# rvolden/C3POa

Hardware: AMD Instinct MI355X
Metric: R2C2 reads->consensus/sec (higher is better)
Workload: dtype int32

## Files before the change

c3poa_amd/_lib.py:

```python
import ctypes as C
import os

import numpy as np

_HERE = os.path.dirname(os.path.abspath(__file__))
LIB_PATH = os.environ.get("C3POA_LIB", os.path.join(_HERE, "lib", "libc3poa_hip.so"))
MAX_PEAKS = 256

STAGE_CONK, STAGE_PEAKS, STAGE_POA, STAGE_POLISH, STAGES_ALL = 1, 2, 4, 8, 15
STAGE_QV = 16
QV_GLOBAL, QV_ANCHOR_START, QV_ANCHOR_END = 0, 1, 2
ST_OK, ST_NOT_ASSIGNED, ST_NO_PEAKS, ST_NO_CONSENSUS, ST_TOO_SHORT, ST_LIMIT = range(6)

EXPORTS = ["c3_default_config", "c3_version", "c3_device_count", "c3_warm_device", "c3_create", "c3_destroy", "c3_last_error", "c3_set_splints",
           "c3_batch_upload", "c3_batch_stage", "c3_batch_commit", "c3_batch_assign", "c3_batch_run", "c3_batch_sync", "c3_batch_results", "c3_batch_results_snapshot", "c3_batch_results_fetch", "c3_batch_timing",
           "c3_fetch_track", "c3_fetch_smoothed", "c3_fetch_raw_peaks", "c3_fetch_draft", "c3_fetch_msa2",
           "c3_call_peaks", "c3_poa_msa", "c3_pairwise_consensus", "c3_determine_consensus", "c3_zero_repeats", "c3_scan_splints",
           "c3_reader_open", "c3_reader_open_range", "c3_reader_close", "c3_reader_error", "c3_reader_names_only", "c3_reader_next", "c3_reader_next_set", "c3_reader_noqual", "c3_reader_reserved_bytes", "c3_reader_range_lost", "c3_write_group",
           "c3_scan_adapters", "c3_match_index", "c3_match_index_batch", "c3_demux_indexes", "c3_demux_host",
           "c3_assign_open", "c3_assign_close", "c3_assign_batch", "c3_assign_seen", "c3_write_splint_psl",
           "c3_host_alloc", "c3_host_free", "c3_writer_reset",
           "c3_batch_results_fetch_qv", "c3_batch_results_qv", "c3_batch_qv_timing", "c3_consensus_qv", "c3_consensus_qv_host",
           "c3_write_consensus_fastq",
           "c3_bgzf_create", "c3_bgzf_destroy", "c3_bgzf_bound", "c3_bgzf_compress", "c3_bgzf_compress_host",
# ... 28 lines not shown
                ("sub_beg", C.c_int32 * MAX_PEAKS), ("sub_end", C.c_int32 * MAX_PEAKS)]


RESULT_DTYPE = np.dtype([("status", "<i4"), ("n_peaks", "<i4"), ("n_sub", "<i4"), ("has_front", "<i4"),
                         ("has_tail", "<i4"), ("front_end", "<i4"), ("tail_beg", "<i4"), ("cons_len", "<i4"),
                         ("draft_len", "<i4"), ("n_win", "<i4"), ("peaks", "<i4", (MAX_PEAKS,)),
                         ("sub_beg", "<i4", (MAX_PEAKS,)), ("sub_end", "<i4", (MAX_PEAKS,))])
assert RESULT_DTYPE.itemsize == C.sizeof(ReadResult)


class Timing(C.Structure):
    _fields_ = [(n, C.c_float) for n in ("ms_pack", "ms_conk", "ms_peaks", "ms_poa", "ms_prep", "ms_window",
                                         "ms_stitch", "ms_total")] + \
               [(n, C.c_int64) for n in ("n_reads", "n_bases", "n_windows", "cells_conk", "cells_poa", "cells_polish", "n_poa_redo")] + \
               [(n, C.c_float) for n in ("ms_wall", "ms_host_worklist", "ms_alloc", "ms_host_gap")] + \
               [(n, C.c_int64) for n in ("cells_polish_computed", "n_band_layers", "n_band_fallback", "n_band_mismatch", "n_win_redo", "n_poa_redo16")]


def _fields_dict(t):
    return {f[0]: getattr(t, f[0]) for f in t._fields_}


class _Info(C.Structure):

    def as_dict(self):
        return {k: int(getattr(self, k)) for k, _t in self._fields_}


class QvTiming(C.Structure):
    _fields_ = [("ms_qv", C.c_float)] + [(n, C.c_int64) for n in ("n_reads", "n_pieces", "n_skipped", "band_cells", "edge_hits")]

# ... 1578 lines not shown
```

c3poa_amd/csrc/c3_args.h:

```cpp
#pragma once
#include "c3_dev.h"
#include <cstddef>

struct C3Counters {
  int queue;
  int peaks_queue;
  unsigned long long cells;
  unsigned long long cells_computed;
  unsigned long long zero_cells;
  int poa_ovf;
  int poa_ovf16;
  int n_windows;
  int win_ovf;
  int win_queue2;
  int band_layers, band_fallback;
  int band_mismatch;
  struct { int window, layer, R, q, band_row, full_row, next_row; } verify;
  unsigned long long phases[16];
};
static_assert(offsetof(C3Counters, cells) % 8 == 0 && offsetof(C3Counters, cells_computed) % 8 == 0 &&
              offsetof(C3Counters, zero_cells) % 8 == 0 && offsetof(C3Counters, phases) % 8 == 0, "u64 counters must be 8-byte aligned");

struct ConkArgs {
  C3Batch b; const uint8_t* sp_codes; const int* sp_len; int32_t* track; C3Info* info; C3Counters* cnt;
  int match, mismatch, penalty;
  int n_spl; int32_t* scan;
};
struct PeaksArgs {
  C3Batch b; const int32_t* track; C3Info* info; double* bufA; double* bufB; int32_t* cand; uint8_t* cstate;
  int32_t* raw_peaks; int32_t* n_raw; const int* sp_len; double coef[64]; int64_t maxL; int window, iters, min_dist;
  C3Counters* cnt;
};
struct PoaArgs {
  C3Batch b; C3Info* info; C3Params p; C3Counters* cnt; const int* work; int n_work;
  int* ibase; int* ebase; char* cellsb; uint8_t* bbase; long long* score;
  int Ncap, K, Pcap, cells_cap;
  uint8_t* draft; int32_t* tpos; uint8_t* msa_dbg; const int64_t* msa_off; int* msa_len;
  int rb_span;
  int no2col;
  uint4* desc; int* jump;
  int* pbase;
  int* overflow;
  int* overflow16;
};
#define C3_POA_NI 19
__host__ __device__ inline int c3_poa_far_shift(bool w32) { return w32 ? 0 : 2; }
struct PoaLayout { size_t ints, edges, cells, bases, score, desc, jump, path, total; };
__host__ __device__ inline PoaLayout c3_poa_layout(size_t Ncap, size_t K, int cells_cap, int far_shift, size_t Pcap) {
  PoaLayout l;
  l.ints = sizeof(int) * C3_POA_NI * Ncap; l.edges = sizeof(int) * 3 * Ncap * K;
  l.cells = 2 * (size_t)cells_cap + 16 * (size_t)(cells_cap >> far_shift);
  l.bases = 5 * Ncap; l.score = sizeof(long long) * Ncap; l.desc = sizeof(uint4) * 2 * Ncap;
  l.jump = sizeof(int) * C3_JUMP_LEVELS * Ncap; l.path = sizeof(int) * Pcap;
  l.total = l.ints + l.edges + l.cells + l.bases + l.score + l.desc + l.jump + l.path;
// ... 69 lines not shown
```

c3poa_amd/csrc/c3_stages.hip:

```cpp
#include "c3_host.h"

__global__ void k_summary(const C3Info* info, const int64_t* off, int n, Summary* out) {
  int i = blockIdx.x * blockDim.x + threadIdx.x;
  if (i >= n) return;
  const C3Info* p = &info[i];
  Summary s; s.status = p->status; s.n_sub = p->n_sub; s.max_sub = 0; s.sum_sub = 0; s.max_dang = 0; s.n_peaks = p->n_peaks;
  for (int k = 0; k < p->n_sub; ++k) { int l = p->sub_end[k] - p->sub_beg[k]; s.sum_sub += l; if (l > s.max_sub) s.max_sub = l; }
  int L = (int)(off[i + 1] - off[i]);
  s.front = p->has_front ? p->front_end : 0; s.tail = p->has_tail ? L - p->tail_beg : 0;
  if (p->has_front) s.max_dang = p->front_end;
  if (p->has_tail && L - p->tail_beg > s.max_dang) s.max_dang = L - p->tail_beg;
  out[i] = s;
}

static hipError_t zero_counters(c3_handle* h) { return hipMemsetAsync(h->d_counter.p, 0, sizeof(C3Counters), h->stream); }

static int auto_slots(c3_handle* h, int want, size_t per_slot_bytes, int n_items, int waves_per_cu) {
  int s = want > 0 ? want : h->n_cus * waves_per_cu;
  size_t budget = h->mem_total ? h->mem_total / 3 : ((size_t)64 << 30);
  if (per_slot_bytes > 0) { size_t mx = budget / per_slot_bytes; if ((size_t)s > mx) s = (int)std::max<size_t>(mx, 1); }
  if (s > n_items) s = std::max(n_items, 1);
  return s;
}

// ... 163 lines not shown
  const PoaLayout L = c3_poa_layout(Ncap, K, (int)cells, c3_poa_far_shift(w32), Pcap);
  const int slots = auto_slots(h, h->cfg.slots_poa, L.total, nw, waves_per_cu);
  const size_t S = (size_t)slots;
  HIPCHK(h->s_poa_i.ensure(L.ints * S)); HIPCHK(h->s_poa_nk.ensure(L.edges * S));
  HIPCHK(h->s_poa_cells.ensure(L.cells * S + 256)); HIPCHK(h->s_poa_b.ensure(L.bases * S)); HIPCHK(h->s_poa_sc.ensure(L.score * S));
  HIPCHK(h->s_poa_desc.ensure(L.desc * S)); HIPCHK(h->s_poa_jump.ensure(L.jump * S)); HIPCHK(h->s_poa_path.ensure(L.path * S));
  PoaArgs a; memset(&a, 0, sizeof(a));
  a.b = dev_batch(h); a.info = h->d_info.as<C3Info>(); a.p = dev_params(h->cfg);
  a.cnt = dev_cnt(h); a.work = d_work; a.n_work = nw;
  a.ibase = h->s_poa_i.as<int>(); a.ebase = h->s_poa_nk.as<int>(); a.cellsb = h->s_poa_cells.as<char>();
  a.bbase = h->s_poa_b.as<uint8_t>(); a.score = h->s_poa_sc.as<long long>();
  a.Ncap = Ncap; a.K = K; a.Pcap = Pcap; a.cells_cap = (int)cells; a.desc = h->s_poa_desc.as<uint4>(); a.jump = h->s_poa_jump.as<int>();
  a.pbase = h->s_poa_path.as<int>(); a.overflow = d_overflow; a.overflow16 = d_overflow16;
  if (const char* e = getenv("C3_DEBUG_POA_RBSPAN")) a.rb_span = std::max(3300, atoi(e));
  a.no2col = getenv("C3_DEBUG_POA_NO2COL") != nullptr;
  a.draft = h->d_draft.as<uint8_t>(); a.tpos = h->d_tpos.as<int32_t>();
  a.msa_dbg = nullptr; a.msa_off = nullptr; a.msa_len = nullptr;
  if (h->debug_msa) { a.msa_dbg = h->d_msa.as<uint8_t>(); a.msa_off = h->d_msa_off.as<int64_t>(); a.msa_len = h->d_msa_len.as<int>(); }
  DBG("poa: nw=%d Ncap=%d K=%d cells=%lld slots=%d (%.1f MB per slot)%s\n", nw, Ncap, K, cells, slots, L.total / 1048576.0, d_overflow ? "" : (d_overflow16 ? " [full-size pass]" : " [32-bit pass]"));
  c3k_launch_poa(&a, slots, w32 ? 1 : 0, wide_ring, h->stream);
  HIPCHK(hipGetLastError());
  return 0;
}

static int run_poa(c3_handle* h) {
  const int nw = (int)h->work.size();
  HIPCHK(h->d_draft.ensure((size_t)h->total + 64)); HIPCHK(h->d_tpos.ensure(sizeof(int32_t) * (size_t)h->total + 64));
  HIPCHK(h->d_cons.ensure((size_t)h->total + 64));
  HIPCHK(hipMemsetAsync(h->d_tpos.p, 0xff, sizeof(int32_t) * (size_t)h->total, h->stream));
  if (nw == 0) return 0;
// ... 7 lines not shown
  const double nodes_typ = (double)max_q * (1.0 + 0.15 * std::max(0, max_ns - 1));
  int Ncap = (int)std::min<double>(Ncap_full, 1.3 * nodes_typ + 256);
  long long cells = std::min<long long>(cells_full, (long long)(1.5 * nodes_typ * (2 * w + 12)) + 4096);
  if (const char* e_ = getenv("C3_DEBUG_POA_SMALL")) { Ncap = std::min(Ncap_full, std::max(64, atoi(e_))); cells = std::min<long long>(cells_full, 16LL * Ncap); }
  if (h->debug_msa) {
    std::vector<int64_t> mo(h->n + 1, 0);
    for (int i = 0; i < h->n; ++i) mo[i + 1] = mo[i] + (int64_t)h->sum[i].n_sub * (h->sum[i].sum_sub + 2);
    HIPCHK(h->d_msa.ensure((size_t)mo[h->n] + 64)); HIPCHK(h->d_msa_off.ensure(sizeof(int64_t) * (h->n + 1))); HIPCHK(h->d_msa_len.ensure(sizeof(int) * h->n));
    HIPCHK(hipMemcpyAsync(h->d_msa_off.p, mo.data(), sizeof(int64_t) * (h->n + 1), hipMemcpyHostToDevice, h->stream));
    HIPCHK(hipMemsetAsync(h->d_msa_len.p, 0, sizeof(int) * h->n, h->stream));
    HIPCHK(hipStreamSynchronize(h->stream));
  }
  HIPCHK(h->d_overflow.ensure(sizeof(int) * 2 * (size_t)nw));
  C3Counters* dc = dev_cnt(h);
  HIPCHK(zero_cnt(h, &dc->queue)); HIPCHK(zero_cnt(h, &dc->cells)); HIPCHK(zero_cnt(h, &dc->poa_ovf)); HIPCHK(zero_cnt(h, &dc->poa_ovf16));
  HIPCHK(zero_cnt(h, &dc->phases));
  int wide_ring = (max_q > 1792 || 2 * w + 1 + 24 > 128) ? 1 : 0;
  if (const char* e_ = getenv("C3_DEBUG_POA_WIDE")) wide_ring = atoi(e_) ? 1 : 0;
  int* ovA = h->d_overflow.as<int>(); int* ovB = h->d_overflow.as<int>() + nw;
  int rc = launch_poa(h, h->d_work.as<int>(), nw, Ncap, K, Pcap, cells, ovA, ovB, 24, wide_ring);
  if (rc) return rc;
  h->n_poa_redo = 0; h->n_poa_redo16 = 0;
  C3Counters c;
  HIPCHK(read_counters(h, &c));
  if (c.poa_ovf > 0) {
    h->n_poa_redo = c.poa_ovf;
    HIPCHK(zero_cnt(h, &dc->queue));
    if ((rc = launch_poa(h, ovA, c.poa_ovf, Ncap_full, K, Pcap, cells_full, nullptr, ovB, 24, wide_ring))) return rc;
    HIPCHK(read_counters(h, &c));
  }
// ... 188 lines not shown
  float ms_prep = 0, ms_win = 0, ms_st = 0;
  if (stages & (C3_STAGE_POA | C3_STAGE_POLISH)) {
    DBG("run: conk+peaks launched\n");
    if ((rc = fetch_summary(h))) return rc;
    DBG("run: work list ready (%zu reads)\n", h->work.size());
    HIPCHK(hipEventRecord(t3, h->stream));
    if (stages & C3_STAGE_POA) {
      if ((rc = run_poa(h))) return rc;
    }
    HIPCHK(hipEventRecord(t4, h->stream));
    if (stages & C3_STAGE_POA) {
      C3Counters c;
      HIPCHK(read_counters(h, &c));
      if (!h->work.empty()) h->tm.cells_poa = (int64_t)(c.zero_cells + c.cells);
      h->tm.n_poa_redo = h->n_poa_redo; h->tm.n_poa_redo16 = h->n_poa_redo16;
      DBG("run: poa done\n");
      HIPCHK(hipEventElapsedTime(&ms, t3, t4)); h->tm.ms_poa = ms;
    }
    if (stages & C3_STAGE_POLISH) { if ((rc = run_polish(h, &ms_prep, &ms_win, &ms_st))) return rc; }
  }
  if (stages & C3_STAGE_QV) { if ((rc = run_qv(h))) return rc; }
  HIPCHK(hipStreamSynchronize(h->stream));
  DBG("run: done\n");
  HIPCHK(hipGetLastError());
  if (stages & C3_STAGE_CONK) { HIPCHK(hipEventElapsedTime(&ms, t0, t1)); h->tm.ms_conk = ms; }
  if (stages & C3_STAGE_PEAKS) { HIPCHK(hipEventElapsedTime(&ms, t1, t2)); h->tm.ms_peaks = ms; }
  if (stages & C3_STAGE_POLISH) { h->tm.ms_prep = ms_prep; h->tm.ms_window = ms_win; h->tm.ms_stitch = ms_st; }
  h->tm.ms_total = h->tm.ms_conk + h->tm.ms_peaks + h->tm.ms_poa + h->tm.ms_prep + h->tm.ms_window + h->tm.ms_stitch;
  h->tm.ms_wall = std::chrono::duration<float, std::milli>(std::chrono::steady_clock::now() - wall0).count();
  h->tm.ms_alloc = (float)(c3h::g_alloc_ms - alloc0);
// ... 6 lines not shown
```

c3poa_amd/csrc/k_poa.hip:

```cpp
#include "c3_dev.h"
#include "c3_args.h"
#include "c3_launch.h"
#include <type_traits>

#define WSYNC() __syncthreads()
#define EI(v, k) ((size_t)(k) * (size_t)c.Ncap + (size_t)(v))
#define SRC 0
#define SNK 1


struct Ctx {
  int* I; int* E; char* C; uint8_t* B8; long long* score_; uint4* desc_; int* jump_; int* path_;
  int K, n, Ncap, cells_cap;
  int far_shift;
  int osel;
  int rb_span;
  int two_col;
  const uint32_t* pk;
#ifdef C3_DEBUG_PUNT
  unsigned long long* dbg;
#endif
#define CTX_I(name, k) __device__ __forceinline__ int* name() const { return I + (size_t)(k) * Ncap; }
  CTX_I(n_in, 0) CTX_I(n_out, 1) CTX_I(grp, 2) CTX_I(index, 5) CTX_I(gfirst, 6) CTX_I(glast, 7)
  CTX_I(rem, 8) CTX_I(mpl, 9) CTX_I(mpr, 10) CTX_I(rowm, 11)  CTX_I(anchor, 14) CTX_I(col, 15)
  CTX_I(col2t, 16) CTX_I(nxt, 17) CTX_I(foff, 18)
#undef CTX_I
  __device__ __forceinline__ int* order() const { return I + (size_t)(3 + osel) * Ncap; }
  __device__ __forceinline__ int* order2() const { return I + (size_t)(4 - osel) * Ncap; }
  __device__ __forceinline__ int* in_from() const { return E; }
  __device__ __forceinline__ int* out_to() const { return E + (size_t)Ncap * K; }
  __device__ __forceinline__ int* out_w() const { return E + 2 * (size_t)Ncap * K; }
  __device__ __forceinline__ int far_cap() const { return cells_cap >> far_shift; }
// ... 120 lines not shown
#endif
__device__ __forceinline__ int maxu16(int a, int b) { int d; asm C3_ASMV("v_max_u16 %0, %1, %2" : "=v"(d) : "v"(a), "v"(b)); return d; }
__device__ __forceinline__ int minu16(int a, int b) { int d; asm C3_ASMV("v_min_u16 %0, %1, %2" : "=v"(d) : "v"(a), "v"(b)); return d; }
__device__ __forceinline__ int cv_16to9(int v, int b8) { return v >= ZLO16 ? (int)((unsigned)(v - BIAS16 + b8) << 6) : NEGS; }
__device__ __forceinline__ int cv_9to16(int x9, int b8, int& bad) {
  if (x9 <= NEGS / 2) return NEG16;
  const int r = (x9 >> 6) - b8 + BIAS16;
  if (r < GLO16 || r > 62000) bad = 1;
  return r;
}


__device__ void poa_sweep_desc(Ctx& c, int lane, int Q, bool qlds, const int PR) {
  const int n = c.n;
  int* hops = c.col();
  for (int c0 = ((n - 1) >> 6) << 6; c0 >= 0; c0 -= 64) {
    const int idx = c0 + lane;
    const bool live = idx < n;
    const int v = live ? c.order()[idx] : SNK;
    const int nin = live ? c.n_in()[v] : 0, nout = live ? c.n_out()[v] : 0;
    int bw = INT32_MIN, bt = SNK;
    unsigned far = 0;
    for (int k = 0; __builtin_amdgcn_ballot_w64(k < nout) != 0; ++k) {
      if (k < nout) {
        const int t = c.out_to()[EI(v, k)], ww = c.out_w()[EI(v, k)];
        if (ww > bw) { bw = ww; bt = t; }
        if (t == SNK || c.index()[t] - idx > PR - 1) far = 1;
      }
    }
    unsigned p[4] = {0, 0, 0, 0};
#pragma unroll
    for (int k = 0; k < 4; ++k) if (k < nin) p[k] = (unsigned)c.index()[c.in_from()[EI(v, k)]];
    int d = (v == SNK) ? 0 : 1, ptr = (v == SNK || !live) ? -1 : c.index()[bt];
    if (ptr >= c0 + 64) { d += hops[ptr]; ptr = -1; }
    for (int r = 0; r < 6 && __builtin_amdgcn_ballot_w64(ptr >= 0) != 0; ++r) {
      const int src = (max(ptr, c0) - c0) << 2;
      const int dd = __builtin_amdgcn_ds_bpermute(src, d), pp = __builtin_amdgcn_ds_bpermute(src, ptr);
      if (ptr >= 0) { d += dd; ptr = pp; }
    }
    if (live) {
      hops[idx] = d;
      uint4 A; A.x = (unsigned)v;
      A.y = (p[0] % PR) | ((p[1] % PR) << 4) | ((p[2] % PR) << 8) | ((p[3] % PR) << 12);
      A.z = (unsigned)c.base()[v] | ((unsigned)min(nin, 255) << 8) | (far << 16) | ((unsigned)(nin > 4) << 17);
      A.z |= ((unsigned)(qlds && nin == 1 && (int)p[0] == idx - 1 && v != SRC && v != SNK) << 18) | ((unsigned)(v == SNK) << 19);
      A.w = (unsigned)(Q - (d - 1));
      uint4 B; B.x = p[0]; B.y = p[1]; B.z = p[2]; B.w = p[3];
      c.descA()[idx] = A; c.descB()[idx] = B;
    }
    WSYNC();
  }
}

template <bool W32, bool DEF, bool WIDE>
__device__ int poa_align(Ctx& c, const C3Params& P, int qb, int Q, int lane, long long* cells PHA) {
  constexpr int PR = WIDE ? 3 : C3_NARROW_PR, PW = WIDE ? C3_WIDE_PW : 128, PWT = PADL + PW + PADR, NCHMAX = PW / 64;
  constexpr int RING_CELLS = WIDE ? RING_CELLS_W : RING_CELLS_N, PQW = WIDE ? PQW_W : PQW_N;
  static_assert(PR * PWT == RING_CELLS, "ring geometry");
  unsigned* const Lqpk = WIDE ? &L.qpk[0] : (unsigned*)&L.ring[3 * RING_CELLS_N];
  const int K = c.K, n = c.n;
// ... 20 lines not shown
    for (int i = lane; i < PQW && from + 16 * i < Q; i += 64) {
      const long long b0 = (long long)qb + from + 16 * i;
      const unsigned w0 = c.pk[b0 >> 4], w1 = c.pk[(b0 >> 4) + 1];
      Lqpk[i] = __builtin_amdgcn_alignbit(w1, w0, (unsigned)(b0 & 15) * 2);
    }
  };
  if (qlds) stage_query(0);
  if (!W32) { unsigned* r32 = (unsigned*)&L.ring[0]; for (int i = lane; i < 3 * RING_CELLS / 2; i += 64) r32[i] = NEG16 | (NEG16 << 16); }
  WSYNC();
  PH_MARK(0)
  int u_beg = 0, u_end = -1, u_left = 0, u_right = 0, u_ncell = 0;
  int u_b8 = 0;
  int u_nfar = 0;
  int pH = NEG16, pE1 = NEG16, pE2 = NEG16;
  bool pv_ok = false;
  int gacc = 0xffff;
  int punt = 0;
  const int lane4 = lane * 4;
  unsigned short* const LH = &L.ring[0]; unsigned short* const LE1 = &L.ring[RING_CELLS]; unsigned short* const LE2 = &L.ring[2 * RING_CELLS];
#ifdef C3_EXP_SBAND
#define UNI(x)
#else
#define UNI(x) asm volatile("" : "+v"(x))
#endif
#ifdef C3_PHASE_PROF
  unsigned long long row_t0 = __builtin_readcyclecounter();
#endif
  int slot = PR - 1;
  for (int ib = 0; ib < n; ib += 64) {
  uint4 dA = c.descA()[min(ib + lane, n - 1)], dB = c.descB()[min(ib + lane, n - 1)];
  asm volatile("" : "+v"(dA.x), "+v"(dA.y), "+v"(dA.z), "+v"(dA.w), "+v"(dB.x), "+v"(dB.y), "+v"(dB.z), "+v"(dB.w));
  const int cnt = min(64, n - ib);
  for (int li = 0; li < cnt; ++li) {
    const int idx = ib + li;
    slot = slot == PR - 1 ? 0 : slot + 1;
    const int fl = __builtin_amdgcn_readlane(dA.z, li);
    if ((fl >> 19) & 1) { pv_ok = false; continue; }
    const int qr = __builtin_amdgcn_readlane(dA.w, li);
    const int vb = fl & 0xff;
    const bool far = W32 || ((fl >> 16) & 1);
    if (WIDE && qr + w + 72 > qwb + PQW * 16 && qwb + PQW * 16 < Q) {
      qwb = max(0, qr - w - 320) & ~15;
      WSYNC(); stage_query(qwb); WSYNC();
    }
#define C3_BAND_OF_ROW_ABOVE \
      UNI(u_beg); UNI(u_end); UNI(u_left); UNI(u_right); UNI(u_ncell); \
      const bool nonempty = u_end >= u_beg; \
      const int mplv = nonempty ? u_left + 1 : INT32_MAX / 2, mprv = nonempty ? u_right + 1 : 0; \
      const int beg = max(max(0, min(mplv, qr) - w), u_beg); \
      int end = min(min(Q, max(mprv, qr) + w), u_end + 1); \
      end = max(end, beg - 1); \
      const int wd = end - beg + 1, sh = beg - u_beg;
    if (!W32 && ((fl >> 18) & 1) && pv_ok) {
      C3_BAND_OF_ROW_ABOVE
      if (__builtin_amdgcn_ballot_w64(((int)((unsigned)(wd - 1) < 64u) & (int)(wd + sh <= 64) & ((int)(sh >= 1) | (int)(u_end - u_beg < 63)) & (int)(u_ncell + 64 <= c.cells_cap) & (int)(!far || u_nfar + 64 <= c.far_cap()) & (int)(!WIDE || (max(beg - 1, 0) >= qwb && end <= qwb + PQW * 16))) != 0) != 0) {
        const int ro = u_ncell;
        const int j = beg + lane;
        const bool act = lane < wd;
        const int jq = max(j - 1, 0) - (WIDE ? qwb : 0);
        const unsigned qw_ = Lqpk[min(jq >> 4, PQW - 1)];
        const int a_p = lane4 + sh * 4, a_d = a_p - 4;
        const int hd = __builtin_amdgcn_ds_bpermute(a_d, pH), hp = __builtin_amdgcn_ds_bpermute(a_p, pH);
        const int e1p = __builtin_amdgcn_ds_bpermute(a_p, pE1), e2p = __builtin_amdgcn_ds_bpermute(a_p, pE2);
        const int qc = (int)((qw_ >> ((jq & 15) * 2)) & 3);
        const int M = hd + ((vb == qc) ? mt8 + 2 : mm8 + 2);
        const int E1t = maxu16(hp - (oe1_8 - 1), e1p - e1_8);
        const int E2t = maxu16(hp - (oe2_8 - 2), e2p - e2_8);
        const int E1c = E1t & ~7, E2c = E2t & ~7;
        const int k2 = maxu16(maxu16(M, E1c + 1), E2c);
        const int ht = k2 & ~7;
// ... 11 lines not shown
        const int rb = __builtin_amdgcn_readlane(s3, 63);
        const unsigned long long mxm = __ballot(htm == rb);
        const int left = beg + __builtin_ctzll(mxm), right = beg + (63 - __builtin_clzll(mxm));
        pH = maxu16(act ? h : NEG16, FLOOR16); pE1 = act ? E1c : NEG16; pE2 = act ? E2c : NEG16;
        int nb8 = u_b8;
        if ((unsigned)(rb - RB_LO16) > (unsigned)c.rb_span) {
          const int m1 = rb - BIAS16, fl1 = FLOOR16 + max(m1, 0);
          nb8 += m1; punt |= (int)(rb < GLO16);
          pH = act ? maxu16(h, fl1) - m1 : NEG16; pE1 = act ? maxu16(E1c, fl1) - m1 : NEG16; pE2 = act ? maxu16(E2c, fl1) - m1 : NEG16;
        }
        gacc = minu16(gacc, pH - (ZHI16 + 1));
#ifdef C3_DEBUG_PUNT
        if (pH > ZHI16 && pH < GLO16) { atomicAdd(c.dbg + 8, 1ull); atomicMax(c.dbg + 9, ((unsigned long long)(65535 - pH) << 40) | ((unsigned long long)idx << 16) | ((unsigned long long)lane << 8) | (unsigned long long)(wd & 255)); atomicMax(c.dbg + 10, ((unsigned long long)(65535 - pH) << 40) | ((unsigned long long)(unsigned short)rb << 16) | (unsigned)(sh & 255) << 8 | (unsigned)(u_end - u_beg + 1)); }
#endif
        c.D8()[(unsigned)(ro + lane)] = (uint8_t)d;
        { const int cb = slot * PWT + PADL + lane;
          LH[cb] = (unsigned short)pH; LE1[cb] = (unsigned short)pE1; LE2[cb] = (unsigned short)pE2;
#pragma unroll
          for (int f = 1; f < NCHMAX; ++f) { LH[cb + 64 * f] = NEG16; LE1[cb + 64 * f] = NEG16; LE2[cb + 64 * f] = NEG16; }
        }
        if (lane == 0) {
          L.meta[slot] = make_int4(beg, end, left, right); L.base8[slot] = nb8;
          int off = 3 * idx; UNI(off);
          int* rm = c.rowm() + off; rm[0] = beg; rm[1] = end; rm[2] = ro;
        }
        if (far) {
          const int fo = wave_first(u_nfar);
          if (act) { c.H()[fo + lane] = cv_16to9(pH, nb8); c.E1()[fo + lane] = cv_16to9(pE1, nb8); c.E2()[fo + lane] = cv_16to9(pE2, nb8); }
          if (lane == 0) { c.mpl()[idx] = left; c.mpr()[idx] = right; c.foff()[idx] = fo; }
          u_nfar = fo + wave_first(wd);
        }
        u_beg = beg; u_end = end; u_left = left; u_right = right; u_ncell = ro + wd; u_b8 = nb8;
#ifdef C3_PHASE_PROF
        { unsigned long long t_ = __builtin_readcyclecounter(); ph_acc_[8] += t_ - row_t0; row_t0 = t_; ph_acc_[12] += 1; }
#endif
        continue;
      }
    }
    if (!WIDE && !W32 && ((fl >> 18) & 1) && c.two_col) {
      C3_BAND_OF_ROW_ABOVE
      if (__builtin_amdgcn_ballot_w64(((int)((unsigned)(wd - 65) < 64u) & (int)((unsigned)(u_end - u_beg) < (unsigned)PW) & (int)(u_ncell + 128 <= c.cells_cap) & (int)(!far || u_nfar + 128 <= c.far_cap())) != 0) != 0) {
        const int ro = u_ncell;
        int c0l = 2 * lane; UNI(c0l);
        const bool act0 = c0l < wd, act1 = c0l + 1 < wd;
        const int j0 = beg + c0l;
        const int jq0 = max(j0 - 1, 0), jq1 = j0;
        const unsigned qw0 = Lqpk[min(jq0 >> 4, PQW - 1)], qw1 = Lqpk[min(jq1 >> 4, PQW - 1)];
        const int rx = (slot == 0 ? PR - 1 : slot - 1) * PWT + PADL + sh + c0l;
        const int hd0 = LH[rx - 1], hp0 = LH[rx], hp1 = LH[rx + 1];
        const int e1p0 = LE1[rx], e1p1 = LE1[rx + 1], e2p0 = LE2[rx], e2p1 = LE2[rx + 1];
        const int qc0 = (int)((qw0 >> ((jq0 & 15) * 2)) & 3), qc1 = (int)((qw1 >> ((jq1 & 15) * 2)) & 3);
        const int M0 = hd0 + ((vb == qc0) ? mt8 + 2 : mm8 + 2), M1 = hp0 + ((vb == qc1) ? mt8 + 2 : mm8 + 2);
        const int E1t0 = maxu16(hp0 - (oe1_8 - 1), e1p0 - e1_8), E1t1 = maxu16(hp1 - (oe1_8 - 1), e1p1 - e1_8);
        const int E2t0 = maxu16(hp0 - (oe2_8 - 2), e2p0 - e2_8), E2t1 = maxu16(hp1 - (oe2_8 - 2), e2p1 - e2_8);
        const int E1c0 = E1t0 & ~7, E2c0 = E2t0 & ~7, E1c1 = E1t1 & ~7, E2c1 = E2t1 & ~7;
        const int k20 = maxu16(maxu16(M0, E1c0 + 1), E2c0), k21 = maxu16(maxu16(M1, E1c1 + 1), E2c1);
// ... 75 lines not shown
#pragma unroll
      for (int k = 0; k < NP; ++k) {
        const bool has = k < nin;
        const int b = has ? m_[k].x : BIGB, e = has ? m_[k].y : -BIGB;
        pb_[k] = b;
        dk_[k] = has ? b8_[k] - b8_[0] : 0;
        dabs = max(dabs, max(dk_[k], -dk_[k]));
        minb = min(minb, b); maxe = max(maxe, e + 1); wmax = max(wmax, e - b);
        const bool ne = e >= b;
        mplv = ne ? min(mplv, m_[k].z + 1) : mplv; mprv = ne ? max(mprv, m_[k].w + 1) : mprv;
      }
      const int beg = max(max(0, min(mplv, qr) - w), minb);
      int end = min(min(Q, max(mprv, qr) + w), maxe);
      end = max(end, beg - 1);
      const int wd = end - beg + 1;
      if (__builtin_amdgcn_ballot_w64(((int)((unsigned)(wd - 1) < (unsigned)(64 * NCH)) & (int)(wmax < PW) & (int)(dabs < 2048) & (int)(u_ncell + 64 * NCH <= c.cells_cap) & (int)(!far || u_nfar + 64 * NCH <= c.far_cap()) & (int)(!WIDE || (max(beg - 1, 0) >= qwb && end <= qwb + PQW * 16))) != 0) == 0) return false;
      const int ro = u_ncell;
      const int W8 = wave_first(b8_[0]);
      int cM[NP], c1o[NP], c1x[NP], c2o[NP], c2x[NP], sb_[NP];
#pragma unroll
      for (int k = 0; k < NP; ++k) {
        cM[k] = dk_[k] + (3 - k);
        c1o[k] = dk_[k] - oe1_8 + (7 - 2 * k); c1x[k] = dk_[k] - e1_8 + (6 - 2 * k);
        c2o[k] = dk_[k] - oe2_8 + (7 - 2 * k); c2x[k] = dk_[k] - e2_8 + (6 - 2 * k);
        sb_[k] = sl_[k] * PWT + PADL - pb_[k];
      }
      int carry1 = 0, carry2 = 0, prev_ht = NEG16;
      int best = 0, left = 0, right = 0;
      int cH[NCH], cE1[NCH], cE2[NCH];
#pragma unroll
      for (int ch = 0; ch < NCH; ++ch) {
// ... 254 lines not shown
        if (c0 + 64 >= wd) { for (int f = 64; c0 + f < PW; f += 64) { LH[cb + f] = NEG16; LE1[cb + f] = NEG16; LE2[cb + f] = NEG16; } }
        if (c0 == 0) { gH = vH; gE1 = vE1; gE2 = vE2; }
      }
      if (cmx > best) { best = cmx; const unsigned long long mm = __ballot(htm == cmx); bl = beg + c0 + __builtin_ctzll(mm); br = beg + c0 + 63 - __builtin_clzll(mm); }
      else if (cmx == best) { const unsigned long long mm = __ballot(htm == cmx); if (mm) br = beg + c0 + 63 - __builtin_clzll(mm); }
    }
    if (!W32 && __builtin_amdgcn_ballot_w64(bad != 0) != 0) punt |= 2;
    const int left = wd > 0 ? bl : 0, right = wd > 0 ? br : 0;
    if (lane == 0) {
      L.meta[slot] = make_int4(beg, end, left, right); L.base8[slot] = Wg;
      { int* rm = c.rowm() + 3 * idx; rm[0] = beg; rm[1] = end | (ty << 28); rm[2] = ro; }
      if (far) { c.mpl()[idx] = left; c.mpr()[idx] = right; }
      if (toglobal || ovf) c.foff()[idx] = fo;
    }
    u_beg = beg; u_end = end; u_left = left; u_right = right; u_ncell = ncell; u_b8 = Wg;
#ifdef C3_PHASE_PROF
    { unsigned long long t_ = __builtin_readcyclecounter(); ph_acc_[11] += t_ - row_t0; row_t0 = t_; }
#endif
    pH = gH; pE1 = gE1; pE2 = gE2; pv_ok = inl && wd <= 64;
  }
  }
  WSYNC();
  *cells += wave_first(u_ncell);
  PH_MARK(1)
#ifdef C3_DEBUG_PUNT
  if (!W32 && lane == 0) { if (punt) atomicAdd(c.dbg + 14, 1ull); if (__builtin_amdgcn_ballot_w64((unsigned)(gacc & 0xffff) < (unsigned)(GLO16 - ZHI16 - 1)) != 0) atomicAdd(c.dbg + 15, 1ull); }
#endif
  if (!W32 && (punt != 0 || __builtin_amdgcn_ballot_w64((unsigned)(gacc & 0xffff) < (unsigned)(GLO16 - ZHI16 - 1)) != 0)) return -5;
  int bi = -1, bs = INT32_MIN;
  for (int k = 0; k < c.n_in()[SNK]; ++k) {
// ... 220 lines not shown
}

#ifndef C3_POA_WAVES
#define C3_POA_WAVES 6
#endif
template <bool W32, bool DEF, bool WIDE>
__global__ __launch_bounds__(64, C3_POA_WAVES) void k_poa(PoaArgs a) {
  const int lane = wave_lane();
  const int slot = blockIdx.x;
  Ctx c;
  const size_t N = (size_t)a.Ncap;
  c.I = a.ibase + (size_t)slot * C3_POA_NI * N; c.path_ = a.pbase + (size_t)slot * a.Pcap; c.E = a.ebase + (size_t)slot * 3 * N * a.K;
  c.far_shift = c3_poa_far_shift(W32);
  c.C = a.cellsb + (size_t)slot * c3_poa_layout(N, a.K, a.cells_cap, c.far_shift, a.Pcap).cells; c.B8 = a.bbase + (size_t)slot * 5 * N;
  c.score_ = a.score + (size_t)slot * N; c.desc_ = a.desc + (size_t)slot * 2 * N; c.jump_ = a.jump + (size_t)slot * C3_JUMP_LEVELS * N;
  c.K = a.K; c.Ncap = a.Ncap; c.cells_cap = a.cells_cap; c.osel = 0; c.rb_span = a.rb_span > 0 ? a.rb_span : RB_HI16 - RB_LO16; c.two_col = !a.no2col;
#ifdef C3_DEBUG_PUNT
  c.dbg = a.cnt->phases;
#endif
  PH_DECL

  for (;;) {
    int wi = 0;
    if (lane == 0) wi = atomicAdd(&a.cnt->queue, 1);
    wi = wave_first(wi);
    if (wi >= a.n_work) break;
    const int rid = a.work[wi];
    C3Info* info = &a.info[rid];
    const int ns = info->n_sub;
    const int64_t off = a.b.off[rid];
    c.pk = a.b.pk + a.b.woff[rid];
    uint8_t* draft = a.draft + off;
    int32_t* tpos = a.tpos + off;
    const uint8_t* qual = a.b.qual + off;
    long long cells = 0;
// ... 166 lines not shown
    const bool to16 = punted || a.overflow == nullptr;
    int* const olist = to16 ? a.overflow16 : a.overflow;
    const bool redo = fail == 2 && olist != nullptr;
    if (lane == 0) {
      if (redo) olist[atomicAdd(to16 ? &a.cnt->poa_ovf16 : &a.cnt->poa_ovf, 1)] = rid;
      else {
        info->draft_len = C;
        if (fail) { info->status = C3_ST_LIMIT; info->draft_len = 0; }
        else if (C == 0) info->status = C3_ST_NO_CONSENSUS;
        atomicAdd(&a.cnt->cells, (unsigned long long)cells);
      }
    }
    WSYNC();
  }
  PH_FLUSH(a.cnt->phases)
}

extern "C" void c3k_launch_poa(const PoaArgs* a, int slots, int wide32, int wide_ring, hipStream_t stream) {
  const C3Params& p = a->p;
  const bool def = p.poa_match == 5 && p.poa_mismatch == 4 && p.o1 == 4 && p.e1 == 2 && p.o2 == 24 && p.e2 == 1;
#define C3_POA_LAUNCH(W, D, R) hipLaunchKernelGGL((k_poa<W, D, R>), dim3(slots), dim3(64), 0, stream, *a)
  if (wide32) { if (def) C3_POA_LAUNCH(true, true, false); else C3_POA_LAUNCH(true, false, false); }
  else if (wide_ring) { if (def) C3_POA_LAUNCH(false, true, true); else C3_POA_LAUNCH(false, false, true); }
  else { if (def) C3_POA_LAUNCH(false, true, false); else C3_POA_LAUNCH(false, false, false); }
#undef C3_POA_LAUNCH
}
```

include/c3poa.h:

```cpp
#ifndef C3POA_H
#define C3POA_H
#include <stdint.h>

#ifdef __cplusplus
extern "C" {
#endif

#define C3_MAX_PEAKS 256

typedef enum {
  C3_E_OK = 0,
  C3_E_NO_DEVICE = -1,
  C3_E_HIP = -2,
  C3_E_ARG = -3,
  C3_E_NOMEM = -4,
  C3_E_STATE = -5,
  C3_E_LIMIT = -6,
  C3_E_DATA = -7
} c3_err;

typedef enum {
  C3_ST_OK = 0,
  C3_ST_NOT_ASSIGNED = 1,
  C3_ST_NO_PEAKS = 2,
// ... 32 lines not shown

typedef struct {
  float ms_pack, ms_conk, ms_peaks, ms_poa, ms_prep, ms_window, ms_stitch, ms_total;
  int64_t n_reads, n_bases, n_windows;
  int64_t cells_conk, cells_poa, cells_polish;
  int64_t n_poa_redo;
  float ms_wall;
  float ms_host_worklist;
  float ms_alloc;
  float ms_host_gap;
  int64_t cells_polish_computed;
  int64_t n_band_layers, n_band_fallback;
  int64_t n_band_mismatch;
  int64_t n_win_redo;
  int64_t n_poa_redo16;
} c3_timing;

typedef struct c3_handle c3_handle;

void c3_default_config(c3_config* cfg);
const char* c3_version(void);
int c3_device_count(void);
int c3_warm_device(int device);

int c3_create(const c3_config* cfg, c3_handle** out);
void c3_destroy(c3_handle* h);
const char* c3_last_error(const c3_handle* h);

int c3_set_splints(c3_handle* h, int n, const char* cat, const int64_t* off);

// ... 263 lines not shown
```

Before: 429,800.

## Skip LDS ring writes for chain rows and precompute block capacity checks

```diff
diff --git a/c3poa_amd/_lib.py b/c3poa_amd/_lib.py
--- a/c3poa_amd/_lib.py
+++ b/c3poa_amd/_lib.py
@@ -66,7 +66,8 @@
                                          "ms_stitch", "ms_total")] + \
                [(n, C.c_int64) for n in ("n_reads", "n_bases", "n_windows", "cells_conk", "cells_poa", "cells_polish", "n_poa_redo")] + \
                [(n, C.c_float) for n in ("ms_wall", "ms_host_worklist", "ms_alloc", "ms_host_gap")] + \
-               [(n, C.c_int64) for n in ("cells_polish_computed", "n_band_layers", "n_band_fallback", "n_band_mismatch", "n_win_redo", "n_poa_redo16")]
+               [(n, C.c_int64) for n in ("cells_polish_computed", "n_band_layers", "n_band_fallback", "n_band_mismatch", "n_win_redo", "n_poa_redo16",
+                                         "n_poa_flush", "n_poa_ring_skips")]
 
 
 def _fields_dict(t):
diff --git a/c3poa_amd/csrc/c3_args.h b/c3poa_amd/csrc/c3_args.h
--- a/c3poa_amd/csrc/c3_args.h
+++ b/c3poa_amd/csrc/c3_args.h
@@ -10,6 +10,8 @@
   unsigned long long zero_cells;
   int poa_ovf;
   int poa_ovf16;
+  unsigned long long poa_flush;
+  unsigned long long poa_skip;
   int n_windows;
   int win_ovf;
   int win_queue2;
@@ -19,7 +21,7 @@
   unsigned long long phases[16];
 };
 static_assert(offsetof(C3Counters, cells) % 8 == 0 && offsetof(C3Counters, cells_computed) % 8 == 0 &&
-              offsetof(C3Counters, zero_cells) % 8 == 0 && offsetof(C3Counters, phases) % 8 == 0, "u64 counters must be 8-byte aligned");
+              offsetof(C3Counters, zero_cells) % 8 == 0 && offsetof(C3Counters, poa_flush) % 8 == 0 && offsetof(C3Counters, phases) % 8 == 0, "u64 counters must be 8-byte aligned");
 
 struct ConkArgs {
   C3Batch b; const uint8_t* sp_codes; const int* sp_len; int32_t* track; C3Info* info; C3Counters* cnt;
@@ -38,6 +40,7 @@
   uint8_t* draft; int32_t* tpos; uint8_t* msa_dbg; const int64_t* msa_off; int* msa_len;
   int rb_span;
   int no2col;
+  int ring_all;
   uint4* desc; int* jump;
   int* pbase;
   int* overflow;
diff --git a/c3poa_amd/csrc/c3_stages.hip b/c3poa_amd/csrc/c3_stages.hip
--- a/c3poa_amd/csrc/c3_stages.hip
+++ b/c3poa_amd/csrc/c3_stages.hip
@@ -201,6 +201,7 @@
   a.pbase = h->s_poa_path.as<int>(); a.overflow = d_overflow; a.overflow16 = d_overflow16;
   if (const char* e = getenv("C3_DEBUG_POA_RBSPAN")) a.rb_span = std::max(3300, atoi(e));
   a.no2col = getenv("C3_DEBUG_POA_NO2COL") != nullptr;
+  a.ring_all = getenv("C3_DEBUG_POA_RINGALL") != nullptr;
   a.draft = h->d_draft.as<uint8_t>(); a.tpos = h->d_tpos.as<int32_t>();
   a.msa_dbg = nullptr; a.msa_off = nullptr; a.msa_len = nullptr;
   if (h->debug_msa) { a.msa_dbg = h->d_msa.as<uint8_t>(); a.msa_off = h->d_msa_off.as<int64_t>(); a.msa_len = h->d_msa_len.as<int>(); }
@@ -238,6 +239,7 @@
   HIPCHK(h->d_overflow.ensure(sizeof(int) * 2 * (size_t)nw));
   C3Counters* dc = dev_cnt(h);
   HIPCHK(zero_cnt(h, &dc->queue)); HIPCHK(zero_cnt(h, &dc->cells)); HIPCHK(zero_cnt(h, &dc->poa_ovf)); HIPCHK(zero_cnt(h, &dc->poa_ovf16));
+  HIPCHK(zero_cnt(h, &dc->poa_flush)); HIPCHK(zero_cnt(h, &dc->poa_skip));
   HIPCHK(zero_cnt(h, &dc->phases));
   int wide_ring = (max_q > 1792 || 2 * w + 1 + 24 > 128) ? 1 : 0;
   if (const char* e_ = getenv("C3_DEBUG_POA_WIDE")) wide_ring = atoi(e_) ? 1 : 0;
@@ -456,6 +458,7 @@
       HIPCHK(read_counters(h, &c));
       if (!h->work.empty()) h->tm.cells_poa = (int64_t)(c.zero_cells + c.cells);
       h->tm.n_poa_redo = h->n_poa_redo; h->tm.n_poa_redo16 = h->n_poa_redo16;
+      h->tm.n_poa_flush = (int64_t)c.poa_flush; h->tm.n_poa_ring_skips = (int64_t)c.poa_skip;
       DBG("run: poa done\n");
       HIPCHK(hipEventElapsedTime(&ms, t3, t4)); h->tm.ms_poa = ms;
     }
diff --git a/c3poa_amd/csrc/k_poa.hip b/c3poa_amd/csrc/k_poa.hip
--- a/c3poa_amd/csrc/k_poa.hip
+++ b/c3poa_amd/csrc/k_poa.hip
@@ -16,6 +16,7 @@
   int osel;
   int rb_span;
   int two_col;
+  int ring_all;
   const uint32_t* pk;
 #ifdef C3_DEBUG_PUNT
   unsigned long long* dbg;
@@ -166,6 +167,7 @@
 __device__ void poa_sweep_desc(Ctx& c, int lane, int Q, bool qlds, const int PR) {
   const int n = c.n;
   int* hops = c.col();
+  int cand_hi = 0;
   for (int c0 = ((n - 1) >> 6) << 6; c0 >= 0; c0 -= 64) {
     const int idx = c0 + lane;
     const bool live = idx < n;
@@ -184,6 +186,9 @@
 #pragma unroll
     for (int k = 0; k < 4; ++k) if (k < nin) p[k] = (unsigned)c.index()[c.in_from()[EI(v, k)]];
     int d = (v == SNK) ? 0 : 1, ptr = (v == SNK || !live) ? -1 : c.index()[bt];
+    const int cand = (int)(live && qlds && nin == 1 && (int)p[0] == idx - 1 && v != SRC && v != SNK);
+    const bool regs_only = nout == 1 && ptr == idx + 1 && wave_shl1(cand, cand_hi) != 0 && !c.ring_all;
+    cand_hi = wave_bcast(cand, 0);
     if (ptr >= c0 + 64) { d += hops[ptr]; ptr = -1; }
     for (int r = 0; r < 6 && __builtin_amdgcn_ballot_w64(ptr >= 0) != 0; ++r) {
       const int src = (max(ptr, c0) - c0) << 2;
@@ -195,7 +200,7 @@
       uint4 A; A.x = (unsigned)v;
       A.y = (p[0] % PR) | ((p[1] % PR) << 4) | ((p[2] % PR) << 8) | ((p[3] % PR) << 12);
       A.z = (unsigned)c.base()[v] | ((unsigned)min(nin, 255) << 8) | (far << 16) | ((unsigned)(nin > 4) << 17);
-      A.z |= ((unsigned)(qlds && nin == 1 && (int)p[0] == idx - 1 && v != SRC && v != SNK) << 18) | ((unsigned)(v == SNK) << 19);
+      A.z |= ((unsigned)cand << 18) | ((unsigned)(v == SNK) << 19) | ((unsigned)!regs_only << 20);
       A.w = (unsigned)(Q - (d - 1));
       uint4 B; B.x = p[0]; B.y = p[1]; B.z = p[2]; B.w = p[3];
       c.descA()[idx] = A; c.descB()[idx] = B;
@@ -246,6 +251,7 @@
   int u_nfar = 0;
   int pH = NEG16, pE1 = NEG16, pE2 = NEG16;
   bool pv_ok = false;
+  bool ring_stale = false;
   int gacc = 0xffff;
   int punt = 0;
   const int lane4 = lane * 4;
@@ -263,11 +269,15 @@
   uint4 dA = c.descA()[min(ib + lane, n - 1)], dB = c.descB()[min(ib + lane, n - 1)];
   asm volatile("" : "+v"(dA.x), "+v"(dA.y), "+v"(dA.z), "+v"(dA.w), "+v"(dB.x), "+v"(dB.y), "+v"(dB.z), "+v"(dB.w));
   const int cnt = min(64, n - ib);
+#define C3_BLOCK_ROOM if (!W32 && __builtin_amdgcn_ballot_w64(((c.cells_cap - 64 * PW - u_ncell) | (c.far_cap() - 64 * PW - u_nfar)) < 0) != 0) dA.z |= 1u << 21;
+#define C3_ROW_ROOM(t, cells) { t |= (c.cells_cap - (cells) - u_ncell) | (far ? c.far_cap() - (cells) - u_nfar : 0); asm volatile("" : "+v"(t)); }
+  C3_BLOCK_ROOM
   for (int li = 0; li < cnt; ++li) {
     const int idx = ib + li;
     slot = slot == PR - 1 ? 0 : slot + 1;
     const int fl = __builtin_amdgcn_readlane(dA.z, li);
-    if ((fl >> 19) & 1) { pv_ok = false; continue; }
+    if ((fl >> 19) & 1) { pv_ok = false; ring_stale = false; continue; }
+    const bool tight = (fl >> 21) & 1;
     const int qr = __builtin_amdgcn_readlane(dA.w, li);
     const int vb = fl & 0xff;
     const bool far = W32 || ((fl >> 16) & 1);
@@ -285,7 +295,10 @@
       const int wd = end - beg + 1, sh = beg - u_beg;
     if (!W32 && ((fl >> 18) & 1) && pv_ok) {
       C3_BAND_OF_ROW_ABOVE
-      if (__builtin_amdgcn_ballot_w64(((int)((unsigned)(wd - 1) < 64u) & (int)(wd + sh <= 64) & ((int)(sh >= 1) | (int)(u_end - u_beg < 63)) & (int)(u_ncell + 64 <= c.cells_cap) & (int)(!far || u_nfar + 64 <= c.far_cap()) & (int)(!WIDE || (max(beg - 1, 0) >= qwb && end <= qwb + PQW * 16))) != 0) != 0) {
+      int qt = (wd - 1) | (u_beg + 63 - end) | ((sh - 1) & (u_beg + 62 - u_end));
+      if (WIDE) qt |= (max(beg - 1, 0) - qwb) | (qwb + PQW * 16 - end);
+      if (tight) C3_ROW_ROOM(qt, 64)
+      if (__builtin_amdgcn_ballot_w64(qt >= 0) != 0) {
         const int ro = u_ncell;
         const int j = beg + lane;
         const bool act = lane < wd;
@@ -327,16 +340,21 @@
         if (pH > ZHI16 && pH < GLO16) { atomicAdd(c.dbg + 8, 1ull); atomicMax(c.dbg + 9, ((unsigned long long)(65535 - pH) << 40) | ((unsigned long long)idx << 16) | ((unsigned long long)lane << 8) | (unsigned long long)(wd & 255)); atomicMax(c.dbg + 10, ((unsigned long long)(65535 - pH) << 40) | ((unsigned long long)(unsigned short)rb << 16) | (unsigned)(sh & 255) << 8 | (unsigned)(u_end - u_beg + 1)); }
 #endif
         c.D8()[(unsigned)(ro + lane)] = (uint8_t)d;
-        { const int cb = slot * PWT + PADL + lane;
-          LH[cb] = (unsigned short)pH; LE1[cb] = (unsigned short)pE1; LE2[cb] = (unsigned short)pE2;
-#pragma unroll
-          for (int f = 1; f < NCHMAX; ++f) { LH[cb + 64 * f] = NEG16; LE1[cb + 64 * f] = NEG16; LE2[cb + 64 * f] = NEG16; }
-        }
         if (lane == 0) {
-          L.meta[slot] = make_int4(beg, end, left, right); L.base8[slot] = nb8;
           int off = 3 * idx; UNI(off);
           int* rm = c.rowm() + off; rm[0] = beg; rm[1] = end; rm[2] = ro;
         }
+        ring_stale = !((fl >> 20) & 1);
+        if (!ring_stale) {
+          const int cb = slot * PWT + PADL + lane;
+          LH[cb] = (unsigned short)pH; LE1[cb] = (unsigned short)pE1; LE2[cb] = (unsigned short)pE2;
+#pragma unroll
+          for (int f = 1; f < NCHMAX; ++f) { LH[cb + 64 * f] = NEG16; LE1[cb + 64 * f] = NEG16; LE2[cb + 64 * f] = NEG16; }
+          if (lane == 0) { L.meta[slot] = make_int4(beg, end, left, right); L.base8[slot] = nb8; }
+        }
+#ifdef C3_PHASE_PROF
+        else if (lane == 0) L.base8[6] = L.base8[6] + 1;
+#endif
         if (far) {
           const int fo = wave_first(u_nfar);
           if (act) { c.H()[fo + lane] = cv_16to9(pH, nb8); c.E1()[fo + lane] = cv_16to9(pE1, nb8); c.E2()[fo + lane] = cv_16to9(pE2, nb8); }
@@ -350,9 +368,20 @@
         continue;
       }
     }
+    if (!W32 && ring_stale) {
+      ring_stale = false;
+      const int pslot = slot == 0 ? PR - 1 : slot - 1;
+      const int cb = pslot * PWT + PADL + lane;
+      LH[cb] = (unsigned short)pH; LE1[cb] = (unsigned short)pE1; LE2[cb] = (unsigned short)pE2;
+#pragma unroll
+      for (int f = 1; f < NCHMAX; ++f) { LH[cb + 64 * f] = NEG16; LE1[cb + 64 * f] = NEG16; LE2[cb + 64 * f] = NEG16; }
+      if (lane == 0) { L.meta[pslot] = make_int4(u_beg, u_end, u_left, u_right); L.base8[pslot] = u_b8; L.base8[7] = L.base8[7] + 1; }
+    }
     if (!WIDE && !W32 && ((fl >> 18) & 1) && c.two_col) {
       C3_BAND_OF_ROW_ABOVE
-      if (__builtin_amdgcn_ballot_w64(((int)((unsigned)(wd - 65) < 64u) & (int)((unsigned)(u_end - u_beg) < (unsigned)PW) & (int)(u_ncell + 128 <= c.cells_cap) & (int)(!far || u_nfar + 128 <= c.far_cap())) != 0) != 0) {
+      int qt = (wd - 65) | (128 - wd) | (u_end - u_beg) | (u_beg + (PW - 1) - u_end);
+      if (tight) C3_ROW_ROOM(qt, 128)
+      if (__builtin_amdgcn_ballot_w64(qt >= 0) != 0) {
         const int ro = u_ncell;
         int c0l = 2 * lane; UNI(c0l);
         const bool act0 = c0l < wd, act1 = c0l + 1 < wd;
@@ -458,7 +487,10 @@
       int end = min(min(Q, max(mprv, qr) + w), maxe);
       end = max(end, beg - 1);
       const int wd = end - beg + 1;
-      if (__builtin_amdgcn_ballot_w64(((int)((unsigned)(wd - 1) < (unsigned)(64 * NCH)) & (int)(wmax < PW) & (int)(dabs < 2048) & (int)(u_ncell + 64 * NCH <= c.cells_cap) & (int)(!far || u_nfar + 64 * NCH <= c.far_cap()) & (int)(!WIDE || (max(beg - 1, 0) >= qwb && end <= qwb + PQW * 16))) != 0) == 0) return false;
+      int qt = (wd - 1) | (64 * NCH - wd) | (PW - 1 - wmax) | (2047 - dabs);
+      if (WIDE) qt |= (max(beg - 1, 0) - qwb) | (qwb + PQW * 16 - end);
+      if (tight) C3_ROW_ROOM(qt, 64 * NCH)
+      if (__builtin_amdgcn_ballot_w64(qt >= 0) == 0) return false;
       const int ro = u_ncell;
       const int W8 = wave_first(b8_[0]);
       int cM[NP], c1o[NP], c1x[NP], c2o[NP], c2x[NP], sb_[NP];
@@ -743,6 +775,7 @@
       if (toglobal || ovf) c.foff()[idx] = fo;
     }
     u_beg = beg; u_end = end; u_left = left; u_right = right; u_ncell = ncell; u_b8 = Wg;
+    C3_BLOCK_ROOM
 #ifdef C3_PHASE_PROF
     { unsigned long long t_ = __builtin_readcyclecounter(); ph_acc_[11] += t_ - row_t0; row_t0 = t_; }
 #endif
@@ -993,11 +1026,12 @@
   c.far_shift = c3_poa_far_shift(W32);
   c.C = a.cellsb + (size_t)slot * c3_poa_layout(N, a.K, a.cells_cap, c.far_shift, a.Pcap).cells; c.B8 = a.bbase + (size_t)slot * 5 * N;
   c.score_ = a.score + (size_t)slot * N; c.desc_ = a.desc + (size_t)slot * 2 * N; c.jump_ = a.jump + (size_t)slot * C3_JUMP_LEVELS * N;
-  c.K = a.K; c.Ncap = a.Ncap; c.cells_cap = a.cells_cap; c.osel = 0; c.rb_span = a.rb_span > 0 ? a.rb_span : RB_HI16 - RB_LO16; c.two_col = !a.no2col;
+  c.K = a.K; c.Ncap = a.Ncap; c.cells_cap = a.cells_cap; c.osel = 0; c.rb_span = a.rb_span > 0 ? a.rb_span : RB_HI16 - RB_LO16; c.two_col = !a.no2col; c.ring_all = a.ring_all;
 #ifdef C3_DEBUG_PUNT
   c.dbg = a.cnt->phases;
 #endif
   PH_DECL
+  if (lane == 0) { L.base8[6] = 0; L.base8[7] = 0; }
 
   for (;;) {
     int wi = 0;
@@ -1194,6 +1228,10 @@
     WSYNC();
   }
   PH_FLUSH(a.cnt->phases)
+  if (lane == 0 && L.base8[7] != 0) atomicAdd(&a.cnt->poa_flush, (unsigned long long)L.base8[7]);
+#ifdef C3_PHASE_PROF
+  if (lane == 0) atomicAdd(&a.cnt->poa_skip, (unsigned long long)L.base8[6]);
+#endif
 }
 
 extern "C" void c3k_launch_poa(const PoaArgs* a, int slots, int wide32, int wide_ring, hipStream_t stream) {
diff --git a/include/c3poa.h b/include/c3poa.h
--- a/include/c3poa.h
+++ b/include/c3poa.h
@@ -70,6 +70,8 @@
   int64_t n_band_mismatch;
   int64_t n_win_redo;
   int64_t n_poa_redo16;
+  int64_t n_poa_flush;
+  int64_t n_poa_ring_skips;
 } c3_timing;
 
 typedef struct c3_handle c3_handle;
```

New measurement: 433,800, median of 6. No clear change (+0.9%).
